# linkedin/ambry

Measured on AMD Instinct MI355X. Metric: GiB/s device-resident CRC32 over 4 MiB blob chunks; % of HBM roofline, higher is better.
Workload: dtype u8; 1 GPU; C3: 8,192 x 4 MiB large-blob router chunks per GPU; chunks_per_gpu=8192, chunk_bytes=4194304, bytes_per_gpu_step=34359738368, parallelism=shard1, kernel_variant=29, grid_workgroups=256, sweep_window_bytes=34359738368

## Files before the change

### ambry_amd/csrc/ambrycrc.cpp

```cpp
#include "../../include/ambrycrc.h"

#include <hip/hip_runtime.h>
#include <stdio.h>
#include <stdlib.h>
#include <string.h>

#include <sched.h>

#include <algorithm>
#include <atomic>
#include <mutex>
#include <string>
#include <thread>
#include <vector>

#include "crc32_gf2.h"
#include "crc32_kernels.h"
#include "crc32_layout.h"
#include "ambrycrc_ctx.h"
#include "host_crc.h"

using namespace ambrycrc;
using namespace ambrycrc::detail;

// ... 177 lines not shown
    } else {
      ++i;
    }
  }
}

int stream_ws(DevCtx* c, hipStream_t s, size_t need, void** out, size_t* entry, bool* capturing_out) {
  hipStreamCaptureStatus cap = hipStreamCaptureStatusNone;
  if (hipStreamIsCapturing(s, &cap) != hipSuccess) return AMBRYCRC_EHIP;
  const bool capturing = cap != hipStreamCaptureStatusNone;
  if (capturing_out) *capturing_out = capturing;
  if (!capturing) reap_retired_ws(c);
  DevCtx::StreamWs* w = nullptr;
  for (auto& e : c->ws_list)
    if (e.stream == s) w = &e;
  if (capturing && (!w || w->bytes < need)) return AMBRYCRC_EINVAL;
  if (capturing) {
    w->captured = true;
    *entry = (size_t)(w - c->ws_list.data());
    *out = w->ptr;
    return AMBRYCRC_OK;
  }
  if (!w && c->ws_list.size() >= kMaxStreamWs) {
    w = &c->ws_list[0];
    for (auto& e : c->ws_list)
      if (e.tick < w->tick) w = &e;
    if (w->ptr && w->captured) {
      c->ws_kept.push_back(w->ptr);
      if (w->last) (void)hipEventDestroy(w->last);
    } else if (w->ptr) {
      if (w->last) {
        c->ws_retired.push_back({w->ptr, w->last});
      } else {
        (void)hipDeviceSynchronize();
        (void)hipFree(w->ptr);
      }
    } else if (w->last) {
      (void)hipEventDestroy(w->last);
    }
    *w = {s, nullptr, 0, nullptr, 0, false};
  }
  if (!w) {
    c->ws_list.push_back({s, nullptr, 0, nullptr, 0, false});
    w = &c->ws_list.back();
  }
  w->tick = ++c->ws_tick;
  *entry = (size_t)(w - c->ws_list.data());
  if (w->bytes >= need) {
    *out = w->ptr;
    return AMBRYCRC_OK;
  }
  if (w->ptr && w->captured) {
    c->ws_kept.push_back(w->ptr);
    w->ptr = nullptr;
    w->captured = false;
  } else if (w->ptr) {
    hipEvent_t ev = nullptr;
    if (hipEventCreateWithFlags(&ev, hipEventDisableTiming) != hipSuccess) return AMBRYCRC_EHIP;
    if (hipEventRecord(ev, s) != hipSuccess) {
      (void)hipEventDestroy(ev);
      return AMBRYCRC_EHIP;
    }
    c->ws_retired.push_back({w->ptr, ev});
    w->ptr = nullptr;
  }
  const size_t sz = std::max(need, w->bytes * 2);
  w->bytes = 0;
  if (hipMalloc(&w->ptr, sz) != hipSuccess) {
    w->ptr = nullptr;
    return AMBRYCRC_ENOMEM;
  }
  w->bytes = sz;
  *out = w->ptr;
  return AMBRYCRC_OK;
}

uint64_t batch_small_max(const DevCtx* c, size_t n) {
  if (n < kGroupMinChunks || !variant_groups(c->variant)) return 0;
  return kGroupSmallMax;
}

int enqueue_batch(DevCtx* c, const uint8_t* base, const uint64_t* off, const uint64_t* len, const uint32_t* crc_in,
                  uint32_t* out, size_t n, void* ws, hipStream_t s, uint32_t* exp_fill, uint8_t* copy_dst,
                  const uint64_t* copy_off, const uint32_t* gate) {
  if (n == 0) return AMBRYCRC_OK;
  PlanArgs p = plan_scan_args(off, len, n, ws, out, gate, crc_in);
  p.small_max = copy_dst ? (n >= kGroupMinChunks ? kGroupSmallMax : 0) : batch_small_max(c, n);
  hipError_t e = launch_plan(p, s);
  if (e != hipSuccess) return AMBRYCRC_EHIP;
  SweepArgs t;
  t.base = base;
  t.off = off;
  t.len = len;
  t.crc_in = p.crc_stage;
  t.n = (uint32_t)n;
  t.byte_start = p.byte_start;
  t.img = c->d_img;
  t.out = out;
  t.small_max = p.small_max;
  t.small_total = p.small_total;
  t.small_idx = p.small_idx;
  t.exp_fill = exp_fill;
  t.window = c->window;
  t.copy_dst = copy_dst;
  t.copy_off = copy_off;
  t.gate = gate;
  if (gate && !copy_dst) return AMBRYCRC_EINVAL;
  EventPair ev{nullptr, nullptr};
  if (c->timing) {
    std::lock_guard<std::mutex> g(c->ev_mu);
    if (!c->free_events.empty()) {
      ev = c->free_events.back();
      c->free_events.pop_back();
    } else if (hipEventCreate(&ev.a) != hipSuccess || hipEventCreate(&ev.b) != hipSuccess) {
      return AMBRYCRC_EHIP;
    }
    if (hipEventRecord(ev.a, s) != hipSuccess) return AMBRYCRC_EHIP;
  }
  e = copy_dst ? launch_sweep_copy(t, c->grid, c->num_cu, c->variant == kVariantSplit ? kVariantSplit : kVariantDefault, s)
               : launch_sweep(t, c->grid, c->num_cu, c->variant, s);
  if (e != hipSuccess) return AMBRYCRC_EHIP;
  if (c->timing) {
    if (hipEventRecord(ev.b, s) != hipSuccess) return AMBRYCRC_EHIP;
    std::lock_guard<std::mutex> g(c->ev_mu);
    c->pending.push_back(ev);
  }
  return AMBRYCRC_OK;
}

void free_ctx(DevCtx* c) {
  if (!c) return;
  (void)hipSetDevice(c->device);
  (void)hipDeviceSynchronize();
  if (c->d_img) (void)hipFree(c->d_img);
  if (c->h_words) (void)hipHostFree(c->h_words);
  for (auto& w : c->ws_list) {
    if (w.ptr) (void)hipFree(w.ptr);
    if (w.last) (void)hipEventDestroy(w.last);
  }
  for (auto& r : c->ws_retired) {
    (void)hipFree(r.ptr);
    (void)hipEventDestroy(r.done);
  }
  for (void* p : c->ws_kept) (void)hipFree(p);
  for (DevCtx::XformSide* x : c->xs_list) {
    if (x->side) (void)hipStreamDestroy(x->side);
    if (x->d_gates) (void)hipFree(x->d_gates);
    if (x->d_done) (void)hipFree(x->d_done);
    if (x->fork) (void)hipEventDestroy(x->fork);
    for (hipEvent_t e : x->ev)
      if (e) (void)hipEventDestroy(e);
    delete x;
  }
  for (auto& e : c->pending) {
    (void)hipEventDestroy(e.a);
    (void)hipEventDestroy(e.b);
  }
  for (auto& e : c->free_events) {
    (void)hipEventDestroy(e.a);
    (void)hipEventDestroy(e.b);
  }
  release_slabs(c);
  delete c;
}

uint32_t fused_proc_waves(const DevCtx* c, size_t m, bool copy) {
  const int waves = copy ? kFusedWavesCopy : kFusedWavesVerify;
  const int most = std::min(kFusedProcMax, waves - 2);
  if (c->fused_proc > 0) return (uint32_t)std::min(c->fused_proc, most);
  const size_t per_cu = m / (size_t)std::max(1, c->num_cu);
  int p;
  if (copy) p = 4;
  else if (per_cu <= 512) p = (int)std::max<size_t>(2, (per_cu + 127) / 128);
  else p = per_cu <= 1024 ? 5 : per_cu <= 1536 ? 6 : per_cu <= 3072 ? 8 : 9;
  return (uint32_t)std::min(p, most);
}

int enqueue_messages(DevCtx* c, const uint8_t* d_region, uint64_t region_len, const uint64_t* d_msg_off, size_t m,
                     uint32_t* d_status, uint64_t* d_msg_end, void* d_ws, size_t ws_bytes, hipStream_t stream) {
  const bool region = c->region_mode && region_len > 0 && region_len <= c->region_max * (uint64_t)m &&
                      msg_jobs_bytes(m) + region_ws_bytes(d_region, region_len, m) <= ws_bytes;
  MsgStage st;
  c->last_msg_mode.store(region ? c->region_mode : 0);
  if (!region) {
    const int rc = enqueue_messages_parse(c, d_region, region_len, d_msg_off, m, d_status, d_msg_end, d_ws, stream, &st);
    return rc ? rc : enqueue_messages_check(c, st, stream);
  }
  st.a.region = d_region;
  st.a.region_len = region_len;
  st.a.msg_off = d_msg_off;
  st.a.m = m;
  st.a.img = c->d_img;
  st.a.status = d_status;
  st.a.msg_end = d_msg_end;
  st.a.inline_max = 0;
  Carver jobs(d_ws);
  msg_jobs(jobs, m, st.a);
  FusedArgs f;
  region_args(c, d_region, region_len, m, jobs.here(), &f);
  Carver k(d_ws);
  long_list(k, jobs.bytes(), f.g.lng);
  if (c->region_mode == 2) {
    const RegionArgs& r = f.g;
// ... 165 lines not shown
  c->device = device;
  c->num_cu = prop.multiProcessorCount;
  c->grid = c->num_cu;
  if (const char* v = getenv("AMBRYCRC_VARIANT")) {
    char* end = nullptr;
    const long x = strtol(v, &end, 10);
    if (end != v && *end == '\0' && x >= 0 && x < 1000 && variant_supported((int)x)) c->variant = (int)x;
  }
  if (const char* v = getenv("AMBRYCRC_REGION")) c->region_mode = strcmp(v, "0") == 0 ? 0 : strcmp(v, "1") == 0 ? 1 : 2;
  if (const char* v = getenv("AMBRYCRC_STREAM_PUT_MAX")) {
    char* end = nullptr;
    const unsigned long x = strtoul(v, &end, 10);
    if (end != v && *end == '\0') c->stream_put_max = x < kStreamPutMax ? x : kStreamPutMax;
  }
  if (const char* v = getenv("AMBRYCRC_XFORM_SIDE")) c->xform_side = strcmp(v, "0") == 0 ? 0 : 1;
  {
    int can = 0;
    if (hipDeviceGetAttribute(&can, hipDeviceAttributeCanUseStreamWaitValue, device) != hipSuccess || !can)
      c->xform_side = 0;
  }
  if (const char* v = getenv("AMBRYCRC_XFORM_FAST_MAX")) {
    char* end = nullptr;
    const unsigned long long x = strtoull(v, &end, 10);
    if (end != v && *end == '\0' && x <= (1ull << 30)) c->xform_fast_max = x;
  }
  if (const char* v = getenv("AMBRYCRC_FUSED_PROC")) {
    char* end = nullptr;
    const long x = strtol(v, &end, 10);
    if (end != v && *end == '\0' && x >= 0 && x <= kFusedProcMax) c->fused_proc = (int)x;
  }
  if (const char* v = getenv("AMBRYCRC_REGION_MAX_PER_MESSAGE")) {
    char* end = nullptr;
    const unsigned long long x = strtoull(v, &end, 10);
    if (end != v && *end == '\0' && x > 0 && x <= (1ull << 30)) c->region_max = x;
  }
  if (const char* v = getenv("AMBRYCRC_XFORM_HOST_VERDICT")) c->xform_host_verdict = strcmp(v, "1") == 0;
  std::vector<uint32_t> img = build_table_image();
  const size_t img_bytes = (img.size() * 4 + 255) & ~size_t(255);
  if (hipMalloc(reinterpret_cast<void**>(&c->d_img), img_bytes + 256) != hipSuccess) {
    delete c;
    return AMBRYCRC_ENOMEM;
  }
  c->d_path = c->d_img + img_bytes / 4;
  if (hipMemcpy(c->d_img, img.data(), img.size() * 4, hipMemcpyHostToDevice) != hipSuccess ||
      hipMemset(c->d_path, 0xFF, 256) != hipSuccess) {
    free_ctx(c);
    return AMBRYCRC_EHIP;
  }
  if (hipHostMalloc(reinterpret_cast<void**>(&c->h_words), DevCtx::kHostWords * sizeof(uint32_t),
                    hipHostMallocDefault) != hipSuccess) {
    c->h_words = nullptr;
    free_ctx(c);
    return AMBRYCRC_ENOMEM;
  }
  g_ctx[device] = c;
  (void)hipSetDevice(prev);
  return AMBRYCRC_OK;
}

int ambrycrc_shutdown(void) {
  std::lock_guard<std::mutex> g(g_mu);
  int prev = 0;
  (void)hipGetDevice(&prev);
  for (int d = 0; d < kMaxDevices; ++d) {
    free_ctx(g_ctx[d]);
    g_ctx[d] = nullptr;
  }
  (void)hipSetDevice(prev);
  return AMBRYCRC_OK;
}

size_t ambrycrc_workspace_bytes(size_t n) { return ws_need(n); }

int ambrycrc_batch_dev(const uint8_t* d_base, const uint64_t* d_off, const uint64_t* d_len, const uint32_t* d_crc_in,
                       uint32_t* d_out, size_t n, void* d_ws, size_t ws_bytes, hipStream_t stream) {
  if (n == 0) return AMBRYCRC_OK;
  if (!d_base || !d_off || !d_len || !d_out || n >= (1ull << 31)) return AMBRYCRC_EINVAL;
  if (!same_or_disjoint(d_crc_in, d_out, n)) return AMBRYCRC_EINVAL;
  DevCtx* c = ctx_current();
  if (!c) return AMBRYCRC_ENOINIT;
  WsLease lease;
  const int rc = lease.acquire(c, stream, &d_ws, ws_bytes, ws_need(n));
  if (rc) return rc;
  return enqueue_batch(c, d_base, d_off, d_len, d_crc_in, d_out, n, d_ws, stream);
}

int ambrycrc_verify_dev(const uint8_t* d_base, const uint64_t* d_off, const uint64_t* d_len, const uint32_t* d_crc_in,
                        const uint32_t* d_expected, uint32_t* d_out, uint8_t* d_mismatch, uint32_t* d_mismatch_count,
                        size_t n, void* d_ws, size_t ws_bytes, hipStream_t stream) {
  if (n == 0) return AMBRYCRC_OK;
  if (!d_base || !d_off || !d_len || !d_expected || n >= (1ull << 31)) return AMBRYCRC_EINVAL;
  if (!same_or_disjoint(d_crc_in, d_out, n)) return AMBRYCRC_EINVAL;
  DevCtx* c = ctx_current();
  if (!c) return AMBRYCRC_ENOINIT;
  Carver need(nullptr);
  verify_scratch(need, n, !d_out);
  WsLease lease;
  int rc = lease.acquire(c, stream, &d_ws, ws_bytes, need.bytes());
  if (rc) return rc;
  Carver k(d_ws);
  if (!d_out) d_out = verify_scratch(k, n, true);
  rc = enqueue_batch(c, d_base, d_off, d_len, d_crc_in, d_out, n, d_ws, stream);
  if (rc) return rc;
  return hip_err(launch_verify(d_out, d_expected, d_mismatch, d_mismatch_count, (uint32_t)n, stream));
}

int ambrycrc_put_crcs(const uint8_t* const* fields, const uint64_t* field_len, const uint8_t* const* prefix,
                      const uint64_t* prefix_len, const uint32_t* blob_crc, const uint64_t* blob_len, size_t n,
                      uint32_t* wire_out, uint32_t* record_out) {
  if (n == 0) return AMBRYCRC_OK;
  if (!blob_crc || !blob_len) return AMBRYCRC_EINVAL;
  if (wire_out && (!fields || !field_len)) return AMBRYCRC_EINVAL;
  if (record_out && (!prefix || !prefix_len)) return AMBRYCRC_EINVAL;
  for (size_t i = 0; i < n; ++i) {
    const uint32_t xb = host_xpow8(blob_len[i]);
    if (wire_out) wire_out[i] = gf2_mul(ambrycrc_update(0, fields[i], field_len[i]), xb) ^ blob_crc[i];
    if (record_out) record_out[i] = gf2_mul(ambrycrc_update(0, prefix[i], prefix_len[i]), xb) ^ blob_crc[i];
  }
  return AMBRYCRC_OK;
}

int ambrycrc_set_variant(int device, int variant) {
  DevCtx* c = ctx_for(device);
  if (!c) return AMBRYCRC_ENOINIT;
  if (!variant_supported(variant)) return AMBRYCRC_EINVAL;
  c->variant = variant;
  return AMBRYCRC_OK;
}

long ambrycrc_set_put_stream_max(int device, long bytes) {
  DevCtx* c = ctx_for(device);
  if (!c) return AMBRYCRC_ENOINIT;
  if (bytes < 0 || (uint64_t)bytes > kStreamPutMax) return AMBRYCRC_EINVAL;
  const long prev = (long)c->stream_put_max;
  c->stream_put_max = (uint64_t)bytes;
  return prev;
}

int ambrycrc_set_region_mode(int device, int enable) {
  DevCtx* c = ctx_for(device);
  if (!c) return AMBRYCRC_ENOINIT;
  if (enable < 0 || enable > 2) return AMBRYCRC_EINVAL;
  c->region_mode = enable;
  return AMBRYCRC_OK;
}


int ambrycrc_get_region_mode(int device) {
  DevCtx* c = ctx_for(device);
  return c ? c->region_mode : AMBRYCRC_ENOINIT;
}

int ambrycrc_last_message_mode(int device) {
  DevCtx* c = ctx_for(device);
  return c ? c->last_msg_mode.load() : AMBRYCRC_ENOINIT;
}

int ambrycrc_last_transform_path(int device) {
  DevCtx* c = ctx_for(device);
  if (!c) return AMBRYCRC_ENOINIT;
  const int p = c->last_xform_path.load();
  if (p != 2) return p;
  uint32_t w = ~0u;
  int prev = 0;
  (void)hipGetDevice(&prev);
  if (hipSetDevice(c->device) != hipSuccess || hipDeviceSynchronize() != hipSuccess ||
      hipMemcpy(&w, c->d_path, sizeof w, hipMemcpyDeviceToHost) != hipSuccess) {
    (void)hipSetDevice(prev);
    return AMBRYCRC_EHIP;
  }
  (void)hipSetDevice(prev);
  return w <= 1 ? (int)w : -1;
}

int ambrycrc_set_transform_verdict(int device, int host) {
  DevCtx* c = ctx_for(device);
  if (!c) return AMBRYCRC_ENOINIT;
  if (host != 0 && host != 1) return AMBRYCRC_EINVAL;
  const int prev = c->xform_host_verdict.exchange(host);
  return prev;
}

int ambrycrc_get_variant(int device) {
  DevCtx* c = ctx_for(device);
  return c ? c->variant : AMBRYCRC_ENOINIT;
// ... 144 lines not shown
```

### ambry_amd/csrc/ambrycrc_ctx.h

```cpp
#pragma once
#include <hip/hip_runtime.h>
#include <stdint.h>
#include <string.h>

#include <atomic>
#include <mutex>
#include <vector>

#include "../../include/ambrycrc.h"
#include "crc32_kernels.h"
#include "ws_layout.h"

namespace ambrycrc {
namespace detail {

constexpr int kMaxDevices = 64;
constexpr int kSlabs = 4;
constexpr size_t kSlabBytes = 64ull << 20;
constexpr size_t kSlabChunks = 1u << 14;

struct EventPair {
  hipEvent_t a, b;
};

// ... 78 lines not shown
  std::atomic<int> last_host_path{-1};
  std::atomic<int> cpu_threads{0};
  static constexpr int kMaxCpuThreads = 256;
  std::atomic<double> cpu_batch_gibps[kMaxCpuThreads + 1];
  DevCtx() {
    for (auto& r : cpu_batch_gibps) r.store(-1.0, std::memory_order_relaxed);
  }
  std::atomic<uint32_t> batch_calls{0};
  std::atomic<double> msg_gpu_gibps[2] = {{44.0}, {22.0}};
  std::atomic<double> msg_cpu_gibps[2] = {{-1.0}, {-1.0}};
  std::atomic<uint32_t> msg_calls[2] = {{0u}, {0u}};
  int fused_proc = AMBRY_FUSED_PROC;
  uint64_t region_max = kRegionMaxPerMessage;
  uint64_t window = 32ull << 30;
  uint32_t* d_img = nullptr;
  struct StreamWs {
    hipStream_t stream;
    void* ptr;
    size_t bytes;
    hipEvent_t last;
    uint64_t tick;
    bool captured;
  };
  struct RetiredWs {
    void* ptr;
    hipEvent_t done;
  };
  std::mutex ws_mu;
  std::vector<StreamWs> ws_list;
  std::vector<RetiredWs> ws_retired;
  std::vector<void*> ws_kept;
  uint64_t ws_tick = 0;
  bool timing = false;
  std::vector<EventPair> pending, free_events;
  bool slabs_ready = false;
  HostSlab slab[kSlabs];
  bool msg_slabs_ready = false;
  MsgSlab msg_slab[kSlabs];
  bool xform_slabs_ready = false;
  XformSlab xform_slab[kSlabs];
  uint64_t last_host_slabs = 0, last_host_oversize = 0;
  std::mutex mu;
  std::mutex ev_mu;
};

int hip_err(hipError_t e);
void release_slabs(DevCtx* c);
int host_cpu_share();
int host_cpu_threads(const DevCtx* c = nullptr);
double host_cpu_gibps(int threads);
bool host_take_cpu(DevCtx* c, int device, int pinned, uint64_t bytes);
void host_note_cpu(DevCtx* c, uint64_t bytes, double seconds);
void host_note_gpu(DevCtx* c, uint64_t bytes, double seconds);
constexpr int kMsgVerify = 0, kMsgTransform = 1;
bool host_take_cpu_msg(DevCtx* c, int device, int pinned, int op, uint64_t bytes);
void host_note_msg(DevCtx* c, int op, bool cpu, uint64_t bytes, double seconds);
double host_msg_cpu_gibps(const DevCtx* c, int op);
DevCtx* ctx_for(int device);
DevCtx* ctx_current();
constexpr size_t kMaxStreamWs = 16;
int stream_ws(DevCtx* c, hipStream_t s, size_t need, void** out, size_t* entry, bool* capturing);
uint64_t batch_small_max(const DevCtx* c, size_t n);
PlanArgs plan_scan_args(const uint64_t* off, const uint64_t* len, size_t n, void* scratch, uint32_t* out,
                        const uint32_t* gate = nullptr, const uint32_t* crc_in = nullptr);
int enqueue_scan_copy(DevCtx* c, const uint64_t* src, const uint64_t* dst_off, const uint64_t* len,
                      const uint64_t* cost, size_t n, uint8_t* dst, void* scratch, uint32_t* out,
                      const uint32_t* gate, hipStream_t s);
inline int enqueue_place(const uint64_t* off, ::ambrycrc_put_desc* desc, uint64_t* out_len, uint64_t* out_off,
                         uint32_t* status, size_t m, uint64_t out_cap, void* scratch, uint32_t* scan_out, hipStream_t s) {
  const PlanArgs p = plan_scan_args(off, out_len, m, scratch, scan_out);
  if (launch_plan(p, s) != hipSuccess) return AMBRYCRC_EHIP;
  TransformArgs t;
  memset(&t, 0, sizeof t);
  t.m = m;
  t.desc = desc;
  t.out_len = out_len;
  t.out_off = out_off;
  t.status = status;
  t.out_cap = out_cap;
  return launch_transform_place(t, p.byte_start, s) == hipSuccess ? AMBRYCRC_OK : AMBRYCRC_EHIP;
}
int enqueue_batch(DevCtx* c, const uint8_t* base, const uint64_t* off, const uint64_t* len, const uint32_t* crc_in,
                  uint32_t* out, size_t n, void* ws, hipStream_t s, uint32_t* exp_fill = nullptr,
                  uint8_t* copy_dst = nullptr, const uint64_t* copy_off = nullptr, const uint32_t* gate = nullptr);

int enqueue_messages(DevCtx* c, const uint8_t* d_region, uint64_t region_len, const uint64_t* d_msg_off, size_t m,
                     uint32_t* d_status, uint64_t* d_msg_end, void* d_ws, size_t ws_bytes, hipStream_t stream);
uint32_t fused_proc_waves(const DevCtx* c, size_t m, bool copy);
void region_args(const DevCtx* c, const uint8_t* d_region, uint64_t region_len, size_t m, void* sums, FusedArgs* f);
struct MsgStage {
  MsgArgs a;
  uint32_t* crc;
  void* batch_ws;
  size_t j;
};
int enqueue_messages_parse(DevCtx* c, const uint8_t* d_region, uint64_t region_len, const uint64_t* d_msg_off,
                           size_t m, uint32_t* d_status, uint64_t* d_msg_end, void* d_ws, hipStream_t stream,
                           MsgStage* st, const TransformArgs* desc = nullptr, const uint32_t* gate = nullptr);
int enqueue_messages_check(DevCtx* c, const MsgStage& st, hipStream_t stream, uint8_t* copy_dst = nullptr,
                           const uint64_t* copy_off = nullptr);
int enqueue_serialize(DevCtx* c, const ::ambrycrc_put_desc* d_desc, size_t m, const uint8_t* d_fields,
                      const uint8_t* d_blobs, uint8_t* d_out, uint64_t* d_msg_len, void* d_ws, hipStream_t stream,
                      const uint32_t* d_in_crc = nullptr, bool layout_only = false, const uint32_t* gate = nullptr,
                      const PropsFix* pfix = nullptr, bool stream_ok = false);

uint64_t message_extent_of(const uint8_t* p, uint64_t rem);
int verify_messages_cpu(const uint8_t* region, uint64_t region_len, const uint64_t* msg_off, size_t m,
                        uint32_t* status, uint64_t* msg_end, int threads);
int transform_messages_cpu(const uint8_t* region, uint64_t region_len, const uint64_t* msg_off, size_t m,
                           const int16_t* life_version, int header_version, uint8_t* out, uint64_t out_cap,
                           uint64_t* out_off, uint64_t* out_len, uint32_t* status, int threads);

struct WsLease {
  std::unique_lock<std::mutex> lk;
  DevCtx* ctx = nullptr;
  hipStream_t stream = nullptr;
  size_t entry = ~size_t(0);
  bool capturing = false;
  int acquire(DevCtx* c, hipStream_t s, void** ws, size_t ws_bytes, size_t need) {
    if (*ws) return ws_bytes < need ? AMBRYCRC_EINVAL : AMBRYCRC_OK;
    lk = std::unique_lock<std::mutex>(c->ws_mu);
    const int rc = stream_ws(c, s, need, ws, &entry, &capturing);
    if (rc == AMBRYCRC_OK) {
      ctx = c;
      stream = s;
    }
    return rc;
  }
  ~WsLease() {
    if (!ctx || capturing || entry >= ctx->ws_list.size()) return;
    DevCtx::StreamWs& w = ctx->ws_list[entry];
    if (!w.last && hipEventCreateWithFlags(&w.last, hipEventDisableTiming) != hipSuccess) w.last = nullptr;
    if (w.last) (void)hipEventRecord(w.last, stream);
  }
};

}
}
```

### ambry_amd/csrc/crc32_kernels.h

```cpp
#pragma once
#include <hip/hip_runtime_api.h>
#include <stdint.h>

#include "../../include/ambrycrc.h"
#include "build_knobs.h"
#include "msg_header.h"

namespace ambrycrc {

struct PropsFix;

struct PlanArgs {
  const uint64_t* off;
  const uint64_t* len;
  const uint32_t* crc_in;
  uint32_t n;
  uint64_t* byte_start;
  uint64_t* block_sum;
  uint32_t* out;
  uint64_t small_max;
  uint64_t* block_small;
  uint64_t* small_total;
  uint32_t* small_idx;
  uint32_t* crc_stage;
  const uint32_t* gate;
};

constexpr uint32_t kPlanPerBlock = AMBRY_PLAN_PER_BLOCK;
static_assert(kPlanPerBlock % 256 == 0 && kPlanPerBlock <= 65535, "plan block size");
constexpr uint64_t kShareQuantum = 1024;
constexpr uint64_t kMinShare = 16384;

struct SweepArgs {
  const uint8_t* base;
  const uint64_t* off;
  const uint64_t* len;
  const uint32_t* crc_in;
  uint32_t n;
  const uint64_t* byte_start;
  const uint32_t* img;
  uint32_t* out;
  uint64_t small_max;
  const uint64_t* small_total;
  const uint32_t* small_idx;
  uint32_t* exp_fill;
  uint64_t window;
  uint8_t* copy_dst;
  const uint64_t* copy_off;
  const uint32_t* gate = nullptr;
};
constexpr uint64_t kCopySkip = ~0ull;

constexpr size_t kGroupMinChunks = 16384;
constexpr uint64_t kGroupSmallMax = 16384;

constexpr int kVariantPieces = 0;
constexpr int kVariantDefault = 29;
constexpr int kVariantSplit = 32;
constexpr bool variant_supported(int v) {
#ifdef AMBRYCRC_DIAGNOSTICS
  if (v >= 100 && v <= 102) return true;
#endif
#ifdef AMBRY_AB_SPLIT_GROUP
  if (v == kVariantSplit) return true;
#endif
  return v == kVariantPieces || v == kVariantDefault;
}
constexpr bool variant_groups(int v) { return v == kVariantDefault || v == kVariantSplit; }
constexpr int kDiagNoFold = 100;

struct LongRec {
  uint64_t pa;
  uint64_t msg;
  uint32_t len, ex;
  uint32_t bit;
  uint32_t piece0;
  uint32_t pieces;
  uint32_t done;
};
struct LongList {
  LongRec* rec = nullptr;
  unsigned long long* ctr = nullptr;
  uint32_t* claim = nullptr;
  uint32_t cap = 0;
  uint32_t* slot = nullptr;
  uint32_t pcap = 0;
};
constexpr uint32_t kLongMaxPieces = 4096;
constexpr uint64_t kLongPiece = 64u << 10;

struct RegionArgs {
  const uint8_t* base;
  uint64_t reg0;
  uint64_t reg_end;
  uint64_t lo16, hi16;
  uint64_t nsb;
  uint32_t* rk;
  const uint32_t* img;
  LongList lng;
};
constexpr uint64_t kRunPad = 32;
constexpr uint64_t kSuperBlock = 4096;
constexpr uint64_t kRegionMaxPerMessage = 6144;
constexpr uint64_t kXformFastMaxPerMessage = 40960;
inline uint64_t region_nsb(const uint8_t* region, uint64_t len) {
  const uint64_t b = reinterpret_cast<uintptr_t>(region) & ~uint64_t(63);
  return (reinterpret_cast<uintptr_t>(region) + len - b + kSuperBlock - 1) / kSuperBlock;
}
inline size_t region_rk_bytes(const uint8_t* region, uint64_t len) {
  return (size_t)((kRunPad + region_nsb(region, len) * 64 + 256) * 4 + 255) & ~size_t(255);
}
inline size_t region_ws_bytes(const uint8_t* region, uint64_t len, uint64_t m) {
  return region_rk_bytes(region, len) + ((256 + 4 * m + 255) & ~size_t(255));
}
hipError_t launch_region_runs(const RegionArgs& a, int grid, hipStream_t s);


struct MsgArgs {
  const uint8_t* region;
  uint64_t region_len;
  const uint64_t* msg_off;
  uint64_t m;
  const uint32_t* img;
  uint64_t* job_off;
  uint64_t* job_len;
  uint32_t* expected;
  const uint32_t* crc;
  uint32_t* status;
  uint64_t* msg_end;
  uint64_t inline_max;
  const uint32_t* gate = nullptr;
};
// ... 173 lines not shown
hipError_t launch_send_finish(const SendArgs& a, int num_cu, hipStream_t s);

struct RecvArgs {
  const uint8_t* body;
  uint64_t body_len;
  const uint64_t* pay_off;
  const uint64_t* pay_size;
  uint64_t m;
  int flag;
  const uint64_t* range;
  const uint64_t* dst_off;
  uint8_t* out;
  uint64_t out_cap;
  ::ambrycrc_recv_info* info;
  uint32_t* status;
  const uint32_t* vstatus;
  const uint64_t* msg_end;
  uint64_t* job_off;
  uint64_t* job_len;
  uint64_t* copy_off;
  const uint32_t* crc;
  uint64_t* len;
  const uint64_t* start;
  const uint32_t* img;
};
hipError_t launch_recv_plan(const RecvArgs& a, int num_cu, hipStream_t s);
hipError_t launch_recv_place(const RecvArgs& a, int num_cu, hipStream_t s);
hipError_t launch_recv_finish(const RecvArgs& a, int num_cu, hipStream_t s);

constexpr uint64_t kStreamPutMax = 6144;
constexpr uint64_t kStreamPutRuns = 100;
struct StreamPutArgs {
  const ::ambrycrc_put_desc* desc;
  uint64_t m;
  uint8_t* obase;
  uint64_t oreg0;
  const uint8_t* fields;
  const uint8_t* blobs;
  uint32_t* rk;
  const uint32_t* img;
};
size_t stream_put_rk_bytes(size_t m);
hipError_t launch_put_stream(const StreamPutArgs& a, int num_cu, hipStream_t s);
hipError_t launch_put_stream_seal(const StreamPutArgs& a, int num_cu, hipStream_t s);

hipError_t launch_put_layout(const PutArgs& a, hipStream_t s);
hipError_t launch_put_seal(const PutArgs& a, hipStream_t s);
hipError_t launch_gather_copy(const CopyArgs& a, int grid, hipStream_t s);

hipError_t launch_trailer_parse(const TrailerArgs& a, hipStream_t s);
hipError_t launch_trailer_verify(const TrailerArgs& a, hipStream_t s);

hipError_t launch_msg_parse(const MsgArgs& a, int num_cu, hipStream_t s);
hipError_t launch_region_msg(const MsgArgs& a, const RegionArgs& g, int num_cu, hipStream_t s);
hipError_t launch_region_long(const MsgArgs& a, const RegionArgs& g, int num_cu, hipStream_t s);
hipError_t launch_msg_reduce(const MsgArgs& a, hipStream_t s);

struct FusedArgs {
  MsgArgs a;
  RegionArgs g;
  uint64_t ngroups;
  uint32_t* ctl;
  uint32_t* defer;
  uint32_t nproc;
  uint8_t* out = nullptr;
  uint64_t out_cap = 0;
  uint64_t* out_off = nullptr;
  uint64_t* out_len = nullptr;
  const int16_t* life = nullptr;
  uint32_t* xstatus = nullptr;
  uint32_t* xfail = nullptr;
  uint64_t* patch = nullptr;
  uint32_t* path_out = nullptr;
};
constexpr uint64_t kGroupBytes = 4 * kSuperBlock;
constexpr uint64_t kDirectSpan = 65536;
constexpr int kFusedWavesVerify = AMBRY_FUSED_WAVES_VERIFY, kFusedWavesCopy = AMBRY_FUSED_WAVES_COPY;
static_assert(kFusedWavesVerify >= 4 && kFusedWavesVerify <= 16 && kFusedWavesCopy >= 4 && kFusedWavesCopy <= 16,
              "one-pass workgroups: 4 to 16 waves (16 run-sum buffers in LDS)");
constexpr int kFusedProcMax = 12;
hipError_t launch_region_fused(const FusedArgs& f, int num_cu, hipStream_t s);

hipError_t launch_plan(const PlanArgs& a, hipStream_t s);
hipError_t launch_sweep(const SweepArgs& a, int grid, int num_cu, int variant, hipStream_t s);
hipError_t launch_sweep_copy(const SweepArgs& a, int grid, int num_cu, int variant, hipStream_t s);
#ifdef AMBRY_AB_SPLIT_GROUP
hipError_t launch_group(const SweepArgs& a, int num_cu, hipStream_t s);
#endif
hipError_t launch_verify(const uint32_t* crc, const uint32_t* expected, uint8_t* mismatch, uint32_t* count,
                         uint32_t n, hipStream_t s);
hipError_t launch_readbw(const uint8_t* base, uint64_t nbytes, uint32_t* out, int grid, int variant,
                         hipStream_t s);
hipError_t launch_fill(uint8_t* dst, uint64_t nbytes, uint64_t seed, uint64_t stream_off, hipStream_t s);

}
```

### ambry_amd/csrc/crc32_kernels.hip

```cpp
#include <hip/hip_runtime.h>
#include <stdint.h>

#include "crc32_gf2.h"
#include "crc32_layout.h"
#include "crc32_kernels.h"
#include "crc_wave.h"
#include "wave_tools.h"

namespace ambrycrc {

template <int DIAG>
__device__ __forceinline__ uint32_t fold(uint32_t s) {
  if constexpr (DIAG == 1) {
    return s ^ (s >> 7);
  } else {
    return nib_mul(s, kFoldOff);
  }
}

template <int DIAG>
__device__ __forceinline__ uint32_t rpiece_pair_d(u32x4 w0, u32x4 w1, const LaneConst& k, uint32_t s) {
  uint32_t x0 = slice4(w0.x, k, w0.y);
  uint32_t x1 = slice4(w1.x, k, w1.y);
  x0 = slice4(x0, k, w0.z);
// ... 583 lines not shown
    i += D;
    if (i >= i1) break;
    r = rn;
    stored = stored_n;
#pragma unroll
    for (uint32_t q = 0; q < BPL; ++q) tb[q] = tbn[q];
    sb = 0;
  }
}

template <int G, int NB, bool NT, bool COPY = false>
__device__ __forceinline__ void group_class(const SweepArgs& a, uint64_t lo, uint64_t hi, uint32_t wave,
                                            uint64_t nwaves, uint32_t lane, const LaneConst& k) {
  constexpr uint32_t S = 64 / G;
  if (hi <= lo) return;
  const GroupRange gr = group_range<G, 0>(lo, hi, wave, nwaves);
  const uint64_t i1 = gr.i1;
  const uint32_t gi = lane / G;
#pragma unroll 1
  for (uint64_t i = gr.i0; i < i1; i += gr.stride) {
    const bool act = i + gi < i1;
    const uint32_t ci = act ? a.small_idx[i + gi] : 0u;
    uint64_t len = 0, off = 0;
    uint32_t cin = 0;
    if (act) {
      len = a.len[ci];
      off = a.off[ci];
      cin = a.crc_in ? a.crc_in[ci] : 0u;
    }
    const uint64_t cb = aligned_end(off, off + len);
    constexpr uint32_t BLK = 16 * G;
    const uint32_t nb = (uint32_t)((cb - off + BLK - 1) / BLK);
    uint32_t nbw = 0;
#pragma unroll
    for (uint32_t q = 0; q < S; ++q) {
      const uint32_t x = __builtin_amdgcn_readlane(nb, q * G);
      nbw = x > nbw ? x : nbw;
    }
    const bool leader = (lane & (G - 1)) == 0 && act;
    uint64_t stored = 0;
    if (a.exp_fill && leader) {
      __builtin_memcpy(&stored, a.base + off + len, 8);
      stored = __builtin_bswap64(stored);
    }
    uint8_t* dbase = nullptr;
    if constexpr (COPY) {
      const uint64_t co = a.copy_off[ci];
      dbase = act && co != kCopySkip ? a.copy_dst + (co - off) : nullptr;
    }
    const uint32_t crc = group_crc_g<G, NB, NT, COPY>(a.base, off, len, cin, nbw, lane, k, dbase);
    if (leader) {
      a.out[ci] = crc;
      if (a.exp_fill) a.exp_fill[ci] = (stored >> 32) ? ~crc : (uint32_t)stored;
    }
  }
}


__device__ __forceinline__ bool group_cls_has_work(const SweepArgs& a, uint32_t first_wave, uint64_t nwaves) {
  const uint64_t c0 = 0, c1 = a.small_total[1], c2 = a.small_total[2], c3 = a.small_total[3];
  const uint64_t c4 = a.small_total[0];
  return (c1 > c0 && group_range<AMBRY_C0_G, 0>(c0, c1, first_wave, nwaves).i0 < c1) ||
         (c2 > c1 && group_range<8, 1>(c1, c2, first_wave, nwaves).i0 < c2) ||
         (c3 > c2 && group_range<16, 2>(c2, c3, first_wave, nwaves).i0 < c3) ||
         (c4 > c3 && group_range<16, 3>(c3, c4, first_wave, nwaves).i0 < c4);
}

template <bool NT, bool COPY = false>
__device__ __forceinline__ void group_phase_cls(const SweepArgs& a, uint32_t wave, uint64_t nwaves, uint32_t lane,
                                                const LaneConst& k) {
  const uint64_t c1 = a.small_total[1], c2 = a.small_total[2], c3 = a.small_total[3], c4 = a.small_total[0];
  group_class<AMBRY_C0_G, AMBRY_C0_NB, NT, COPY>(a, 0, c1, wave, nwaves, lane, k);
  group_class_t4s<8, 1, NT, COPY>(a, c1, c2, wave, nwaves, lane, k);
  group_class_t4s<16, 2, NT, COPY>(a, c2, c3, wave, nwaves, lane, k);
  group_class_t4s<16, 3, NT, COPY>(a, c3, c4, wave, nwaves, lane, k);
}

__device__ __forceinline__ uint64_t snap_cut(uint64_t cs, uint64_t len, uint64_t r) {
  const uint64_t a = (cs + r + 15) & ~uint64_t(15);
  const uint64_t rr = a - cs;
  return rr < len ? rr : len;
}

template <bool T4, bool GROUP, int DIAG = 0, bool COPY = false>
__global__ __launch_bounds__(1024) void crc32_sweep_kernel(SweepArgs a) {
  static_assert(!COPY || (T4 && DIAG == 0), "copy-through is built for the 64-B-run sweep only");
  if (COPY && a.gate && *a.gate == 0) return;
  const uint32_t waves_per_block = blockDim.x >> 6;
  const uint64_t nwaves = (uint64_t)gridDim.x * waves_per_block;
  const uint64_t total = a.byte_start[a.n];
  uint64_t share = ((total + nwaves - 1) / nwaves + kShareQuantum - 1) & ~uint64_t(kShareQuantum - 1);
  share = share < kMinShare ? kMinShare : share;
  const uint64_t ns = GROUP ? *a.small_total : 0;
  const bool grp = GROUP && ns > 0 && group_cls_has_work(a, blockIdx.x, nwaves);
  if ((uint64_t)blockIdx.x * share >= total && !grp) return;
  fill_lds(a.img);

  const uint32_t lane = threadIdx.x & 63u;
  const uint32_t wave = __builtin_amdgcn_readfirstlane((threadIdx.x >> 6) * gridDim.x + blockIdx.x);
  if constexpr (GROUP) {
    if (grp) group_phase_cls<true, COPY>(a, wave, nwaves, lane, make_lane_const(lane));
  }
  uint64_t S = share;
  uint64_t round_step = 0;
  if (a.window && total > a.window) {
    const uint64_t R = (total + a.window - 1) / a.window;
    S = ((total + R * nwaves - 1) / (R * nwaves) + kShareQuantum - 1) & ~uint64_t(kShareQuantum - 1);
    S = S < kMinShare ? kMinShare : S;
    round_step = nwaves * S;
  }
  uint64_t g0 = (uint64_t)wave * S;
  if (g0 >= total) return;
  uint64_t g1 = g0 + S < total ? g0 + S : total;
  const uint32_t* xpow2 = a.img + kLdsBytes / 4;
  const LaneConst k = make_lane_const(lane);

  uint64_t init_len = ~0ull;
  uint32_t init_term = 0;

  auto segment = [&](uint64_t bsc, uint64_t len, uint64_t cs, uint32_t cin, uint64_t dsh, bool* whole) -> uint32_t {
    const uint64_t ce = cs + len;
    const uint64_t cb = aligned_end(cs, ce);
    const uint64_t r0 = g0 > bsc ? snap_cut(cs, len, g0 - bsc) : 0;
    const uint64_t r1 = g1 - bsc < len ? snap_cut(cs, len, g1 - bsc) : len;
    *whole = r0 == 0 && r1 == len;
    if (r0 >= r1) return 0u;
    const uint64_t sa = cs + r0, se = cs + r1;
    const uint64_t be = se == ce ? cb : se;
    uint32_t r = 0;
    if (sa < be) {
      if constexpr (T4) {
        r = body_crc_t4<1, true, true, COPY>(a.base, sa, be, lane, k, reinterpret_cast<uint8_t*>(dsh));
      } else {
        r = body_crc<8, true, DIAG>(a.base, sa, be, lane, k);
      }
      r = __builtin_amdgcn_readlane(r, 63);
      r = shift_bytes(r, ce - be, xpow2);
    }
    if (se == ce && ce > cb) {
      const uint64_t t0 = sa > cb ? sa : cb;
      r ^= __builtin_amdgcn_readlane(tail_crc(a.base + t0, (uint32_t)(ce - t0), lane), 0);
      if constexpr (COPY) {
        if (dsh && lane < ce - t0) st8g(reinterpret_cast<uint8_t*>(dsh) + t0 + lane, a.base[t0 + lane]);
      }
    }
    if (r0 == 0) {
      if (cin == 0) {
        if (len != init_len) {
          init_term = shift_bytes(0xFFFFFFFFu, len, xpow2) ^ 0xFFFFFFFFu;
          init_len = len;
        }
        r ^= init_term;
      } else {
        r ^= shift_bytes(~cin, len, xpow2) ^ 0xFFFFFFFFu;
      }
    }
    return r;
  };
  auto emit_partial = [&](uint32_t ci, uint32_t r) {
    if constexpr (DIAG == 2) {
      if (lane == 0 && r == 0x9E3779B9u) a.out[ci] = r;
    } else {
      if (lane == 0) atomicXor(&a.out[ci], r);
    }
  };

  for (;;) {
    uint32_t c = __builtin_amdgcn_readfirstlane(find_start(a.byte_start, a.n, g0, lane));
    bool done = false;
    while (!done && c < a.n) {
      const uint32_t cnt = a.n - c < 64u ? a.n - c : 64u;
      uint64_t w_bs = ~0ull, w_len = 0, w_off = 0, w_dst = 0;
      uint32_t w_cin = 0;
      if (lane < cnt) {
        w_bs = a.byte_start[c + lane];
        w_len = a.len[c + lane];
        w_off = a.off[c + lane];
        w_cin = a.crc_in ? a.crc_in[c + lane] : 0u;
        if constexpr (COPY) {
          const uint64_t co = a.copy_off[c + lane];
          w_dst = co == kCopySkip ? 0 : (uint64_t)(uintptr_t)a.copy_dst + co - w_off;
        }
      }
      uint64_t bsc = readlane64(w_bs, 0);
      bool work = false;
      for (uint32_t j = 0; j < cnt;) {
        if (bsc >= g1) {
          done = true;
          break;
        }
        const uint64_t len = readlane64(w_len, j);
        const uint64_t span = len > a.small_max ? len : 0;
        if (span != 0) {
          work = true;
          bool whole;
          const uint32_t r = segment(bsc, len, readlane64(w_off, j), __builtin_amdgcn_readlane(w_cin, j),
                                     COPY ? readlane64(w_dst, j) : 0, &whole);
          if (whole && DIAG != 2) {
            if (lane == 0) a.out[c + j] = r;
          } else {
            emit_partial(c + j, r);
          }
        }
        bsc += span;
        ++j;
      }
      uint32_t next = c + cnt;
      if (!work && !done && next < a.n) {
        const uint32_t far = __builtin_amdgcn_readfirstlane(find_start(a.byte_start, a.n, bsc, lane));
        next = far > next ? far : next;
      }
      c = next;
    }
    if (round_step == 0) break;
    g0 += round_step;
    if (g0 >= total) break;
    g1 = g0 + S < total ? g0 + S : total;
  }
}

__device__ __forceinline__ uint64_t wave_scan64(uint64_t v) {
#define AMBRY_SCAN_STEP(C, R)                                  \
  {                                                            \
    const uint32_t lo = dpp<C, R>((uint32_t)v);                \
    const uint32_t hi = dpp<C, R>((uint32_t)(v >> 32));        \
    v += ((uint64_t)hi << 32) | lo;                            \
  }
  AMBRY_SCAN_STEP(0x111, 0xf)
  AMBRY_SCAN_STEP(0x112, 0xf)
  AMBRY_SCAN_STEP(0x114, 0xf)
  AMBRY_SCAN_STEP(0x118, 0xf)
  AMBRY_SCAN_STEP(0x142, 0xa)
  AMBRY_SCAN_STEP(0x143, 0xc)
#undef AMBRY_SCAN_STEP
  return v;
}

template <int N>
__device__ __forceinline__ void block_scan256(uint64_t (&v)[N], uint64_t (&total)[N]) {
  __shared__ uint64_t wsum[4][N];
  const uint32_t lane = threadIdx.x & 63u, wv = threadIdx.x >> 6;
#pragma unroll
  for (int i = 0; i < N; ++i) {
    v[i] = wave_scan64(v[i]);
    if (lane == 63) wsum[wv][i] = v[i];
  }
  __syncthreads();
#pragma unroll
  for (int i = 0; i < N; ++i) {
    uint64_t before = 0;
    for (uint32_t w = 0; w < wv; ++w) before += wsum[w][i];
    total[i] = wsum[0][i] + wsum[1][i] + wsum[2][i] + wsum[3][i];
    v[i] += before;
  }
  __syncthreads();
}

__device__ __forceinline__ uint64_t share_len(uint64_t len, uint64_t small_max) {
  return len > small_max ? len : 0u;
}

__device__ __forceinline__ bool is_small(uint64_t len, uint64_t small_max) { return len != 0 && len <= small_max; }

__device__ __forceinline__ uint32_t small_class(uint64_t len) {
  return len <= 256 ? 0u : len <= AMBRY_C1_MAX ? 1u : len <= 4096 ? 2u : 3u;
}
__device__ __forceinline__ uint64_t class_onehot(uint64_t len, uint64_t small_max) {
  return is_small(len, small_max) ? (1ull << (16 * small_class(len))) : 0ull;
}
__device__ __forceinline__ uint64_t field16(uint64_t v, uint32_t c) { return (v >> (16 * c)) & 0xFFFFu; }

__global__ __launch_bounds__(256) void crc32_plan_count_kernel(PlanArgs a) {
  if (a.gate && *a.gate == 0) return;
  const uint32_t base = blockIdx.x * kPlanPerBlock;
  uint64_t len[kPlanPerBlock / 256];
#pragma unroll
  for (uint32_t r = 0; r < kPlanPerBlock / 256; ++r) {
    const uint32_t c = base + r * 256 + threadIdx.x;
    len[r] = c < a.n ? a.len[c] : 0u;
  }
  uint64_t v[2] = {0, 0}, total[2];
#pragma unroll
  for (uint32_t r = 0; r < kPlanPerBlock / 256; ++r) {
    v[0] += share_len(len[r], a.small_max);
    v[1] += class_onehot(len[r], a.small_max);
  }
  block_scan256<2>(v, total);
  if (threadIdx.x == 0) {
    a.block_sum[blockIdx.x] = total[0];
    a.block_small[blockIdx.x] = total[1];
  }
}

__global__ __launch_bounds__(256) __attribute__((amdgpu_waves_per_eu(5))) void crc32_plan_scan_kernel(PlanArgs a) {
  if (a.gate && *a.gate == 0) return;
  constexpr uint32_t R = kPlanPerBlock / 256;
  constexpr uint32_t P = R + 1;
  __shared__ uint64_t lds[256 * P];
// ... 84 lines not shown
    b += share_len(ln, a.small_max);
    if (is_small(ln, a.small_max)) {
      const uint32_t k = small_class(ln);
      const uint64_t p = k == 0 ? pos[0] : k == 1 ? pos[1] : k == 2 ? pos[2] : pos[3];
      a.small_idx[p] = c;
#pragma unroll
      for (uint32_t q = 0; q < 4; ++q) pos[q] += q == k ? 1u : 0u;
    }
    if (c == a.n - 1) a.byte_start[a.n] = b;
  }
  const bool store_starts = a.small_max == 0 || (nblocks > 1 ? __syncthreads_or(any_share) != 0 : tot[5] != 0);
  __syncthreads();
  if (store_starts) {
#pragma unroll
    for (uint32_t r = 0; r < R; ++r) {
      const uint32_t i = r * 256 + tid, c = base + i;
      if (c < a.n) a.byte_start[c] = lds[(i / R) * P + i % R];
    }
  }
  if (blockIdx.x == 0 && tid == 0) {
    a.small_total[4] = 0;
    a.small_total[0] = cls_base[3] + cls_total[3];
    a.small_total[1] = cls_base[1];
    a.small_total[2] = cls_base[2];
    a.small_total[3] = cls_base[3];
  }
}

__global__ void crc32_verify_kernel(const uint32_t* __restrict__ crc, const uint32_t* __restrict__ expected,
                                    uint8_t* __restrict__ mismatch, uint32_t* __restrict__ count, uint32_t n) {
  const uint32_t i = blockIdx.x * blockDim.x + threadIdx.x;
  if (i >= n) return;
  const bool bad = crc[i] != expected[i];
  if (mismatch) mismatch[i] = bad ? 1 : 0;
  if (bad && count) atomicAdd(count, 1u);
}

__device__ __forceinline__ uint64_t splitmix_mix(uint64_t z) {
  z = (z ^ (z >> 30)) * 0xBF58476D1CE4E5B9ull;
  z = (z ^ (z >> 27)) * 0x94D049BB133111EBull;
  return z ^ (z >> 31);
}

__global__ void fill_splitmix_kernel(uint8_t* __restrict__ dst, uint64_t nbytes, uint64_t seed, uint64_t stream_off) {
  const uint64_t n16 = nbytes / 16;
  const uint64_t stride = (uint64_t)gridDim.x * blockDim.x;
  for (uint64_t i = (uint64_t)blockIdx.x * blockDim.x + threadIdx.x; i < n16; i += stride) {
    const uint64_t word = (stream_off >> 3) + 2 * i;
    const uint64_t w0 = splitmix_mix(seed + (word + 1) * 0x9E3779B97F4A7C15ull);
    const uint64_t w1 = splitmix_mix(seed + (word + 2) * 0x9E3779B97F4A7C15ull);
    u32x4 v = {(uint32_t)w0, (uint32_t)(w0 >> 32), (uint32_t)w1, (uint32_t)(w1 >> 32)};
    reinterpret_cast<u32x4*>(dst)[i] = v;
  }
  if (blockIdx.x == 0 && threadIdx.x < (nbytes & 15)) {
    const uint64_t pos = stream_off + n16 * 16 + threadIdx.x;
    const uint64_t w = splitmix_mix(seed + ((pos >> 3) + 1) * 0x9E3779B97F4A7C15ull);
    dst[n16 * 16 + threadIdx.x] = (uint8_t)(w >> (8 * (pos & 7)));
  }
}

hipError_t launch_plan(const PlanArgs& a, hipStream_t s) {
  const uint32_t blocks = blocks_for(a.n, 0, 0, kPlanPerBlock);
  if (blocks > 1) hipLaunchKernelGGL(crc32_plan_count_kernel, dim3(blocks), dim3(256), 0, s, a);
  return launch_items(crc32_plan_scan_kernel, blocks, 256, s, a);
}

hipError_t launch_sweep_copy(const SweepArgs& a, int grid, int num_cu, int variant, hipStream_t s) {
#ifdef AMBRY_AB_SPLIT_GROUP
  if (variant == kVariantSplit) {
    if (a.small_max) {
      const hipError_t e = launch_group(a, num_cu, s);
      if (e != hipSuccess) return e;
    }
    hipLaunchKernelGGL((crc32_sweep_kernel<true, false, 0, true>), dim3(grid), dim3(1024), 0, s, a);
    return hipGetLastError();
  }
#endif
  (void)variant;
  (void)num_cu;
  hipLaunchKernelGGL((crc32_sweep_kernel<true, true, 0, true>), dim3(grid), dim3(1024), 0, s, a);
  return hipGetLastError();
}

hipError_t launch_sweep(const SweepArgs& a, int grid, int num_cu, int variant, hipStream_t s) {
  (void)num_cu;
  switch (variant) {
    case kVariantPieces: hipLaunchKernelGGL((crc32_sweep_kernel<false, false>), dim3(grid), dim3(1024), 0, s, a); break;
    case kVariantDefault: hipLaunchKernelGGL((crc32_sweep_kernel<true, true>), dim3(grid), dim3(1024), 0, s, a); break;
#ifdef AMBRY_AB_SPLIT_GROUP
    case kVariantSplit:
      if (a.small_max) {
        const hipError_t e = launch_group(a, num_cu, s);
        if (e != hipSuccess) return e;
      }
      hipLaunchKernelGGL((crc32_sweep_kernel<true, false>), dim3(grid), dim3(1024), 0, s, a);
      break;
#endif
#ifdef AMBRYCRC_DIAGNOSTICS
    case kDiagNoFold: hipLaunchKernelGGL((crc32_sweep_kernel<false, false, 1>), dim3(grid), dim3(1024), 0, s, a); break;
    case kDiagNoFold + 1: hipLaunchKernelGGL((crc32_sweep_kernel<false, false, 2>), dim3(grid), dim3(1024), 0, s, a); break;
    case kDiagNoFold + 2: hipLaunchKernelGGL((crc32_sweep_kernel<false, false, 3>), dim3(grid), dim3(1024), 0, s, a); break;
#endif
    default: return hipErrorInvalidValue;
  }
  return hipGetLastError();
}

hipError_t launch_verify(const uint32_t* crc, const uint32_t* expected, uint8_t* mismatch, uint32_t* count,
                         uint32_t n, hipStream_t s) {
  return launch_items(crc32_verify_kernel, blocks_for(n), 256, s, crc, expected, mismatch, count, n);
}

hipError_t launch_fill(uint8_t* dst, uint64_t nbytes, uint64_t seed, uint64_t stream_off, hipStream_t s) {
  if (nbytes == 0) return hipSuccess;
  uint64_t n16 = nbytes / 16;
  uint64_t blocks = (n16 + 255) / 256;
  if (blocks > 65536) blocks = 65536;
  if (blocks == 0) blocks = 1;
  hipLaunchKernelGGL(fill_splitmix_kernel, dim3((uint32_t)blocks), dim3(256), 0, s, dst, nbytes, seed, stream_off);
  return hipGetLastError();
}

}
```

Measured before the change: 6117 GiB/s.

## Split windowed sweep into paired launch with atomic ticket work-stealing rounds

For device batch and verify calls on the default variant with a sweep window, the sweep now issues two kernels. The first handles the small-group pass and exits its large-byte work when the total exceeds the window. The second, a ticket instance, walks the large bytes in smaller rounds (capped at 8 GiB), and each wave claims its next share through a global atomic counter instead of a fixed stride. The aim is to balance load dynamically across waves and reduce tail imbalance. In exchange it adds an extra launch, atomic contention, and relies on a ticket slot in the workspace being zeroed, which the plan step is presumably expected to do.

```diff
diff --git a/ambry_amd/csrc/ambrycrc.cpp b/ambry_amd/csrc/ambrycrc.cpp
--- a/ambry_amd/csrc/ambrycrc.cpp
+++ b/ambry_amd/csrc/ambrycrc.cpp
@@ -283,7 +283,7 @@
 
 int enqueue_batch(DevCtx* c, const uint8_t* base, const uint64_t* off, const uint64_t* len, const uint32_t* crc_in,
                   uint32_t* out, size_t n, void* ws, hipStream_t s, uint32_t* exp_fill, uint8_t* copy_dst,
-                  const uint64_t* copy_off, const uint32_t* gate) {
+                  const uint64_t* copy_off, const uint32_t* gate, bool paired) {
   if (n == 0) return AMBRYCRC_OK;
   PlanArgs p = plan_scan_args(off, len, n, ws, out, gate, crc_in);
   p.small_max = copy_dst ? (n >= kGroupMinChunks ? kGroupSmallMax : 0) : batch_small_max(c, n);
@@ -306,6 +306,7 @@
   t.copy_dst = copy_dst;
   t.copy_off = copy_off;
   t.gate = gate;
+  t.ticket = paired && !copy_dst ? p.small_total + 4 : nullptr;
   if (gate && !copy_dst) return AMBRYCRC_EINVAL;
   EventPair ev{nullptr, nullptr};
   if (c->timing) {
@@ -319,7 +320,7 @@
     if (hipEventRecord(ev.a, s) != hipSuccess) return AMBRYCRC_EHIP;
   }
   e = copy_dst ? launch_sweep_copy(t, c->grid, c->num_cu, c->variant == kVariantSplit ? kVariantSplit : kVariantDefault, s)
-               : launch_sweep(t, c->grid, c->num_cu, c->variant, s);
+               : launch_sweep(t, c->grid, c->num_cu, c->variant, s, paired);
   if (e != hipSuccess) return AMBRYCRC_EHIP;
   if (c->timing) {
     if (hipEventRecord(ev.b, s) != hipSuccess) return AMBRYCRC_EHIP;
@@ -651,7 +652,8 @@
   WsLease lease;
   const int rc = lease.acquire(c, stream, &d_ws, ws_bytes, ws_need(n));
   if (rc) return rc;
-  return enqueue_batch(c, d_base, d_off, d_len, d_crc_in, d_out, n, d_ws, stream);
+  return enqueue_batch(c, d_base, d_off, d_len, d_crc_in, d_out, n, d_ws, stream, nullptr, nullptr, nullptr, nullptr,
+                       true);
 }
 
 int ambrycrc_verify_dev(const uint8_t* d_base, const uint64_t* d_off, const uint64_t* d_len, const uint32_t* d_crc_in,
@@ -669,7 +671,8 @@
   if (rc) return rc;
   Carver k(d_ws);
   if (!d_out) d_out = verify_scratch(k, n, true);
-  rc = enqueue_batch(c, d_base, d_off, d_len, d_crc_in, d_out, n, d_ws, stream);
+  rc = enqueue_batch(c, d_base, d_off, d_len, d_crc_in, d_out, n, d_ws, stream, nullptr, nullptr, nullptr, nullptr,
+                     true);
   if (rc) return rc;
   return hip_err(launch_verify(d_out, d_expected, d_mismatch, d_mismatch_count, (uint32_t)n, stream));
 }
diff --git a/ambry_amd/csrc/ambrycrc_ctx.h b/ambry_amd/csrc/ambrycrc_ctx.h
--- a/ambry_amd/csrc/ambrycrc_ctx.h
+++ b/ambry_amd/csrc/ambrycrc_ctx.h
@@ -184,7 +184,8 @@
 }
 int enqueue_batch(DevCtx* c, const uint8_t* base, const uint64_t* off, const uint64_t* len, const uint32_t* crc_in,
                   uint32_t* out, size_t n, void* ws, hipStream_t s, uint32_t* exp_fill = nullptr,
-                  uint8_t* copy_dst = nullptr, const uint64_t* copy_off = nullptr, const uint32_t* gate = nullptr);
+                  uint8_t* copy_dst = nullptr, const uint64_t* copy_off = nullptr, const uint32_t* gate = nullptr,
+                  bool paired = false);
 
 int enqueue_messages(DevCtx* c, const uint8_t* d_region, uint64_t region_len, const uint64_t* d_msg_off, size_t m,
                      uint32_t* d_status, uint64_t* d_msg_end, void* d_ws, size_t ws_bytes, hipStream_t stream);
diff --git a/ambry_amd/csrc/crc32_kernels.h b/ambry_amd/csrc/crc32_kernels.h
--- a/ambry_amd/csrc/crc32_kernels.h
+++ b/ambry_amd/csrc/crc32_kernels.h
@@ -30,6 +30,7 @@
 static_assert(kPlanPerBlock % 256 == 0 && kPlanPerBlock <= 65535, "plan block size");
 constexpr uint64_t kShareQuantum = 1024;
 constexpr uint64_t kMinShare = 16384;
+constexpr uint64_t kTicketRound = 8ull << 30;
 
 struct SweepArgs {
   const uint8_t* base;
@@ -48,6 +49,7 @@
   uint8_t* copy_dst;
   const uint64_t* copy_off;
   const uint32_t* gate = nullptr;
+  uint64_t* ticket = nullptr;
 };
 constexpr uint64_t kCopySkip = ~0ull;
 
@@ -387,7 +389,7 @@
 hipError_t launch_region_fused(const FusedArgs& f, int num_cu, hipStream_t s);
 
 hipError_t launch_plan(const PlanArgs& a, hipStream_t s);
-hipError_t launch_sweep(const SweepArgs& a, int grid, int num_cu, int variant, hipStream_t s);
+hipError_t launch_sweep(const SweepArgs& a, int grid, int num_cu, int variant, hipStream_t s, bool paired = false);
 hipError_t launch_sweep_copy(const SweepArgs& a, int grid, int num_cu, int variant, hipStream_t s);
 #ifdef AMBRY_AB_SPLIT_GROUP
 hipError_t launch_group(const SweepArgs& a, int num_cu, hipStream_t s);
diff --git a/ambry_amd/csrc/crc32_kernels.hip b/ambry_amd/csrc/crc32_kernels.hip
--- a/ambry_amd/csrc/crc32_kernels.hip
+++ b/ambry_amd/csrc/crc32_kernels.hip
@@ -689,16 +689,21 @@
   return rr < len ? rr : len;
 }
 
-template <bool T4, bool GROUP, int DIAG = 0, bool COPY = false>
+template <bool T4, bool GROUP, int DIAG = 0, bool COPY = false, bool TICKET = false>
 __global__ __launch_bounds__(1024) void crc32_sweep_kernel(SweepArgs a) {
+  if (TICKET && !(a.window && a.byte_start[a.n] > a.window)) return;
   static_assert(!COPY || (T4 && DIAG == 0), "copy-through is built for the 64-B-run sweep only");
+  static_assert(!TICKET || (T4 && GROUP && DIAG == 0 && !COPY), "the ticket instance is variant 29's, read-only");
+  constexpr bool PAIRABLE = T4 && GROUP && DIAG == 0 && !COPY && !TICKET;
   if (COPY && a.gate && *a.gate == 0) return;
   const uint32_t waves_per_block = blockDim.x >> 6;
   const uint64_t nwaves = (uint64_t)gridDim.x * waves_per_block;
-  const uint64_t total = a.byte_start[a.n];
+  uint64_t total = a.byte_start[a.n];
+  const bool other = PAIRABLE && a.ticket && a.window && total > a.window;
+  if (other) total = 0;
   uint64_t share = ((total + nwaves - 1) / nwaves + kShareQuantum - 1) & ~uint64_t(kShareQuantum - 1);
   share = share < kMinShare ? kMinShare : share;
-  const uint64_t ns = GROUP ? *a.small_total : 0;
+  const uint64_t ns = GROUP && !other ? *a.small_total : 0;
   const bool grp = GROUP && ns > 0 && group_cls_has_work(a, blockIdx.x, nwaves);
   if ((uint64_t)blockIdx.x * share >= total && !grp) return;
   fill_lds(a.img);
@@ -711,7 +716,8 @@
   uint64_t S = share;
   uint64_t round_step = 0;
   if (a.window && total > a.window) {
-    const uint64_t R = (total + a.window - 1) / a.window;
+    const uint64_t round = TICKET && a.window > kTicketRound ? kTicketRound : a.window;
+    const uint64_t R = (total + round - 1) / round;
     S = ((total + R * nwaves - 1) / (R * nwaves) + kShareQuantum - 1) & ~uint64_t(kShareQuantum - 1);
     S = S < kMinShare ? kMinShare : S;
     round_step = nwaves * S;
@@ -820,7 +826,13 @@
       c = next;
     }
     if (round_step == 0) break;
-    g0 += round_step;
+    if constexpr (TICKET) {
+      uint64_t t = 0;
+      if (lane == 0) t = atomicAdd(reinterpret_cast<unsigned long long*>(a.ticket), 1ull);
+      g0 = round_step + readlane64(t, 0) * S;
+    } else {
+      g0 += round_step;
+    }
     if (g0 >= total) break;
     g1 = g0 + S < total ? g0 + S : total;
   }
@@ -1071,8 +1083,15 @@
   return hipGetLastError();
 }
 
-hipError_t launch_sweep(const SweepArgs& a, int grid, int num_cu, int variant, hipStream_t s) {
+hipError_t launch_sweep(const SweepArgs& args, int grid, int num_cu, int variant, hipStream_t s, bool paired) {
   (void)num_cu;
+  SweepArgs a = args;
+  if (paired && variant == kVariantDefault && a.window != 0 && a.ticket) {
+    hipLaunchKernelGGL((crc32_sweep_kernel<true, true>), dim3(grid), dim3(1024), 0, s, a);
+    hipLaunchKernelGGL((crc32_sweep_kernel<true, true, 0, false, true>), dim3(grid), dim3(1024), 0, s, a);
+    return hipGetLastError();
+  }
+  a.ticket = nullptr;
   switch (variant) {
     case kVariantPieces: hipLaunchKernelGGL((crc32_sweep_kernel<false, false>), dim3(grid), dim3(1024), 0, s, a); break;
     case kVariantDefault: hipLaunchKernelGGL((crc32_sweep_kernel<true, true>), dim3(grid), dim3(1024), 0, s, a); break;
```

Result: no change. 6116 GiB/s (-0.0%).
